# francis0407/streaming-benchmarks

Hardware: AMD Instinct MI355X
Metric: events/sec (parse+filter+join+window count) at 1/8 GPUs; % HBM roofline (higher is better)
Workload: dtype u8; 1 GPU; configs[1]: 100M JSON events per GPU, 100 campaigns x 10 ads, 10 s windows; events_per_gpu=100000000, campaigns=100, ads=1000, parallelism=1 GPU

## Files before the change

### streaming-benchmarks_amd/csrc/ysb_capi.cpp

```cpp
#include "ysb_ctx.h"

#include <unistd.h>

#include <cctype>

using namespace ysb;

thread_local std::string g_open_err;

int fail(ysb_ctx* c, int code, const char* fmt, ...) {
    char buf[1024];
    va_list ap;
    va_start(ap, fmt);
    vsnprintf(buf, sizeof buf, fmt, ap);
    va_end(ap);
    if (c) c->err = buf;
    else g_open_err = buf;
    return code;
}

int grow_device(ysb_ctx* c, DevMem& buf, u64 bytes, u64 floor_bytes) {
    if (buf.bytes() >= bytes) return YSB_OK;
    for (hipStream_t s : {c->s_comp, c->s_copy, c->s_split, c->s_x})
        if (s) HIPCHK(c, hipStreamSynchronize(s));
// ... 72 lines not shown
    c->max_ads = 1000;
    c->max_batch_events = 1u << 20;
    c->max_batch_bytes = 256ull << 20;
    c->ring_base_bucket = INT64_MIN;
    c->overflow_capacity = 1u << 20;
    c->flags = 0;
}

const char* ysb_last_error(const ysb_ctx* c) { return c ? c->err.c_str() : g_open_err.c_str(); }

static void destroy(ysb_ctx* c) {
    if (!c) return;
    hipSetDevice(c->device);
    for (hipStream_t s : {c->s_comp, c->s_copy, c->s_split, c->s_x})
        if (s) hipStreamSynchronize(s);
    if (c->comm) ncclCommDestroy(c->comm);
    for (auto& r : c->host_ranges) hipHostUnregister(reinterpret_cast<void*>(r.first));
    if (c->s_x) hipStreamDestroy(c->s_x);
    if (c->s_split) hipStreamDestroy(c->s_split);
    if (c->s_comp) hipStreamDestroy(c->s_comp);
    if (c->s_copy) hipStreamDestroy(c->s_copy);
    delete c;
}

static int init(ysb_ctx* c) {
    const ysb_config& cfg = c->cfg;
    if (hipSetDevice(c->device) != hipSuccess) return fail(c, YSB_ERR_HIP, "hipSetDevice(%d) failed", c->device);
    hipDeviceProp_t prop;
    if (hipGetDeviceProperties(&prop, c->device) == hipSuccess && prop.multiProcessorCount > 0) c->cus = prop.multiProcessorCount;
    if (const char* e = getenv("YSB_DYN_PCT")) c->dyn_pct = (u32)strtoul(e, nullptr, 10);
    if (const char* e = getenv("YSB_DELTA_FOLD_EVENTS")) {
        const u64 v = strtoull(e, nullptr, 10);
        if (v > 0 && v < c->delta_limit) c->delta_limit = v;
    }
    if (const char* e = getenv("YSB_DYN_CHUNK")) c->dyn_chunk = (u32)strtoul(e, nullptr, 10);
    if (const char* e = getenv("YSB_SPLIT_STREAM")) c->split_place = std::atoi(e);
    if (const char* e = getenv("YSB_H2D_WG")) c->h2d_wg = std::max(1, std::atoi(e));
    if (const char* e = getenv("YSB_H2D_PRIO")) c->h2d_prio = std::atoi(e) != 0;
    if (const char* e = getenv("YSB_H2D_GRID")) c->h2d_grid = std::max(0, std::atoi(e));
    if (hipStreamCreateWithFlags(&c->s_comp, hipStreamNonBlocking) != hipSuccess ||
        hipStreamCreateWithFlags(&c->s_copy, hipStreamNonBlocking) != hipSuccess)
        return fail(c, YSB_ERR_HIP, "stream creation failed");
    for (Event* e : {&c->ev_h2d[0], &c->ev_kdone[0], &c->ev_h2d[1], &c->ev_kdone[1], &c->ev_ring, &c->ev_used})
        if (e->create() != hipSuccess) return fail(c, YSB_ERR_HIP, "event creation failed");
    if (c->h_used.alloc(16) != hipSuccess) return fail(c, YSB_ERR_HIP, "event creation failed");
    const int rc = regrow_table(c, c->d_counts, 0, (u64)c->c_pad * cfg.window_ring);
    if (rc) return rc;
    c->side_slots = 64;
    while (c->side_slots < 2 * cfg.overflow_capacity) c->side_slots <<= 1;
    c->side_cbits = 1;
    while (c->side_cbits < 32 && (1ull << c->side_cbits) <= cfg.n_campaigns) ++c->side_cbits;
    if (c->d_side.alloc(c->side_slots * sizeof(SideSlot)) != hipSuccess ||
        c->d_stats.alloc((ST_COUNT_ + 1) * 8) != hipSuccess ||
        hipMemset(c->d_stats, 0, (ST_COUNT_ + 1) * 8) != hipSuccess ||
        c->d_dirty.alloc(16) != hipSuccess || hipMemset(c->d_dirty, 0, 16) != hipSuccess)
        return fail(c, YSB_ERR_NOMEM, "device allocation failed");
    c->d_side_used = reinterpret_cast<u32*>(c->d_stats + ST_COUNT_);
    launch_side_clear(c->d_side, c->side_slots, c->s_comp);
    if (hipStreamSynchronize(c->s_comp) != hipSuccess) return fail(c, YSB_ERR_HIP, "side map initialisation failed");
    if (c->d_ring.alloc(16) != hipSuccess || c->h_ring.alloc(16) != hipSuccess ||
        c->d_ovf.alloc(cfg.overflow_capacity * sizeof(OvfEntry)) != hipSuccess || c->d_ovf_count.alloc(16) != hipSuccess)
        return fail(c, YSB_ERR_NOMEM, "device allocation failed");
    i64 ring[2] = {0, 0};
    if (cfg.ring_base_bucket != INT64_MIN) {
        ring[0] = cfg.ring_base_bucket;
        ring[1] = 1;
// ... 570 lines not shown
```

### streaming-benchmarks_amd/csrc/ysb_count.hip

```cpp
#include "ysb_kernels.h"
#include <algorithm>

namespace ysb {

constexpr int REC_TPB = 1024;
constexpr int PART_RING = 32;
constexpr int REC_WAVES = REC_TPB / 64;
constexpr int REC_UNROLL = 8;
constexpr u32 REC_NONE = 0xFFFFFFFFu;

__global__ __launch_bounds__(REC_TPB) __attribute__((amdgpu_waves_per_eu(PART_RING == 32 ? 8 : 4)))
void rec_partition_kernel(const RecParams R) {
    __shared__ __attribute__((aligned(16))) u32 stage[REC_SUB_MAX * PART_RING];
    __shared__ u32 hist[REC_SUB_MAX];
    __shared__ u32 boff[REC_SUB_MAX];
    __shared__ u32 cur[REC_SUB_MAX];
    __shared__ u32 fl[REC_SUB_MAX];
    __shared__ u32 rounds_sh;
    const u32 tid = threadIdx.x, lane = tid & 63, wave = tid >> 6;
    const u32 b = blockIdx.x / REC_QUARTERS, q = blockIdx.x % REC_QUARTERS;
    const u32 S = 1u << R.sub_log2;
    for (u32 i = tid; i < S; i += REC_TPB) { hist[i] = 0; cur[i] = 0; fl[i] = 0; }
    if (tid == 0) rounds_sh = 0;
    const u32 w_lo = (u32)((u64)q * R.grid / REC_QUARTERS), w_hi = (u32)((u64)(q + 1) * R.grid / REC_QUARTERS);
    const u32 first_blk = b << R.sub_log2;
    const u32 sh = R.w_log2 + R.blk_shift;
    constexpr u32 CH = 64 * REC_UNROLL;
    u32 my_rounds = 0;
    for (u32 w = w_lo + wave; w < w_hi; w += REC_WAVES) my_rounds += (R.rec_n[(u64)w * R.bins + b] + CH - 1) / CH;
    __syncthreads();
    if (lane == 0) atomicMax(&rounds_sh, my_rounds);
    u32 cw = w_lo + wave, coff = 0, cn = cw < w_hi ? R.rec_n[(u64)cw * R.bins + b] : 0u;
    auto next_chunk = [&](u32 (&v)[REC_UNROLL]) {
        while (cw < w_hi && coff >= cn) {
            cw += REC_WAVES;
            coff = 0;
            cn = cw < w_hi ? R.rec_n[(u64)cw * R.bins + b] : 0u;
        }
        const u32* src = R.rec + ((u64)(cw < w_hi ? cw : w_lo) * R.bins + b) * R.cap;
#pragma unroll
        for (int u = 0; u < REC_UNROLL; ++u) {
            const u32 i = coff + u * 64 + lane;
// ... 49 lines not shown
            for (u32 j = 0; j < n; ++j) dst[j] = src[(f + j) & (PART_RING - 1)];
        }
        fl[k] = f + n;
    };
    cw = w_lo + wave;
    coff = 0;
    cn = cw < w_hi ? R.rec_n[(u64)cw * R.bins + b] : 0u;
    for (u32 r = 0; r < rounds; ++r) {
        if (r < my_rounds) {
            u32 v[REC_UNROLL];
            next_chunk(v);
#pragma unroll
            for (int u = 0; u < REC_UNROLL; ++u) {
                if (v[u] == REC_NONE) continue;
                const u32 k = (v[u] >> sh) - first_blk;
                const u32 pos = atomicAdd(&cur[k], 1u);
                if (pos - fl[k] < (u32)PART_RING) stage[k * PART_RING + (pos & (PART_RING - 1))] = v[u];
                else out[boff[k] + pos] = v[u];
            }
        }
        __syncthreads();
        for (u32 k = tid; k < S; k += REC_TPB) {
            const u32 f0 = fl[k], c = cur[k];
            const u32 lines = min(c - f0, (u32)PART_RING) / 32;
            for (u32 l = 0; l < lines; ++l) write_line(k, 32);
            if (c - f0 > (u32)PART_RING) fl[k] = c;
        }
        __syncthreads();
    }
    for (u32 k = tid; k < S; k += REC_TPB)
        if (cur[k] > fl[k]) write_line(k, cur[k] - fl[k]);
}

__device__ __forceinline__ uint4 add16(uint4 d, const u32* cnt16, unsigned long long* ring16, u32* dirty) {
    const u32 dw[4] = {d.x, d.y, d.z, d.w};
    u32 o[4];
#pragma unroll
    for (int k = 0; k < 4; ++k) {
        const uint4 c = reinterpret_cast<const uint4*>(cnt16)[k];
        const u32 cc[4] = {c.x, c.y, c.z, c.w};
        u32 w = 0;
#pragma unroll
        for (int j = 0; j < 4; ++j) {
            const u32 s = ((dw[k] >> (8 * j)) & 0xFFu) + cc[j];
            if (s > 255u) {
                atomicAdd(&ring16[4 * k + j], (unsigned long long)s);
                *dirty = 1u;
            } else {
                w |= s << (8 * j);
            }
        }
        o[k] = w;
    }
    return make_uint4(o[0], o[1], o[2], o[3]);
}

__global__ __launch_bounds__(REC_TPB) void rec_count_kernel(const RecParams R) {
    __shared__ __attribute__((aligned(16))) u32 cnt[REC_BLOCK_CELLS];
    __shared__ u32 roff[REC_QUARTERS + 1];
    __shared__ u32 rbeg[REC_QUARTERS];
    const u32 tid = threadIdx.x;
    const u32 j = blockIdx.x;
    const u32 c0 = j << R.blk_shift;
    const u32 nc = min(1u << R.blk_shift, R.c_pad - c0);
    const u32 cells = nc << R.w_log2;
    for (u32 i = tid; i < cells / 4; i += REC_TPB) reinterpret_cast<uint4*>(cnt)[i] = make_uint4(0, 0, 0, 0);
    if (tid < 64) {
        const u32 n = tid < (u32)REC_QUARTERS ? R.runs[((u64)j * REC_QUARTERS + tid) * 2 + 1] : 0u;
        if (tid < (u32)REC_QUARTERS) rbeg[tid] = R.runs[((u64)j * REC_QUARTERS + tid) * 2];
        u32 incl = n;
#pragma unroll
        for (int o = 1; o < 64; o <<= 1) {
            const u32 y = __shfl_up(incl, o, 64);
            if ((int)tid >= o) incl += y;
        }
        if (tid < (u32)REC_QUARTERS) roff[tid] = incl - n;
        if (tid == (u32)REC_QUARTERS - 1) roff[REC_QUARTERS] = incl;
    }
    __syncthreads();
    const u32 total = roff[REC_QUARTERS];
    const u32 base_cell = c0 << R.w_log2;
    uint4* dr = reinterpret_cast<uint4*>(R.delta + base_cell);
    const u32 quads = cells / 16;
    constexpr int SU = REC_BLOCK_CELLS / 16 / REC_TPB;
    static_assert(SU * REC_TPB * 16 == REC_BLOCK_CELLS, "one slab vector set per thread");
    unsigned long long* ring = R.counts + base_cell;
    const bool dense = (u64)total * 16u >= cells;
    uint4 r[SU];
    if (dense) {
#pragma unroll
        for (int u = 0; u < SU; ++u) {
            const u32 p = u * REC_TPB + tid;
            r[u] = p < quads ? dr[p] : make_uint4(0u, 0u, 0u, 0u);
        }
    }
    constexpr u32 TPS = REC_TPB / REC_QUARTERS;
    static_assert(TPS * REC_QUARTERS == REC_TPB && TPS >= 16, "one thread group per partition slice");
    const u32 q = tid / TPS, k = tid % TPS;
    const u32 nq = roff[q + 1] - roff[q];
    const u32* src = R.part + rbeg[q];
    for (u32 j0 = 0; j0 < nq; j0 += TPS * REC_UNROLL) {
        u32 v[REC_UNROLL];
#pragma unroll
        for (int u = 0; u < REC_UNROLL; ++u) {
            const u32 jj = j0 + u * TPS + k;
            v[u] = jj < nq ? src[jj] : REC_NONE;
        }
#pragma unroll
        for (int u = 0; u < REC_UNROLL; ++u)
            if (v[u] != REC_NONE) atomicAdd(&cnt[v[u] - base_cell], 1u);
    }
    __syncthreads();
    if (dense) {
#pragma unroll
        for (int u = 0; u < SU; ++u) {
            const u32 p = u * REC_TPB + tid;
            if (p < quads) dr[p] = add16(r[u], cnt + 16 * p, ring + 16 * (u64)p, R.dirty);
        }
        return;
    }
    bool live[SU];
#pragma unroll
    for (int u = 0; u < SU; ++u) {
        const u32 p = u * REC_TPB + tid;
        u32 any = 0;
        if (p < quads) {
#pragma unroll
            for (int j = 0; j < 4; ++j) {
                const uint4 c = reinterpret_cast<const uint4*>(cnt)[4 * p + j];
                any |= c.x | c.y | c.z | c.w;
            }
        }
        any |= __shfl_xor(any, 1, 64);
        any |= __shfl_xor(any, 2, 64);
        any |= __shfl_xor(any, 4, 64);
        live[u] = p < quads && any != 0u;
    }
#pragma unroll
    for (int u = 0; u < SU; ++u) {
        const u32 p = u * REC_TPB + tid;
        if (live[u]) r[u] = dr[p];
    }
#pragma unroll
    for (int u = 0; u < SU; ++u) {
        const u32 p = u * REC_TPB + tid;
        if (live[u]) dr[p] = add16(r[u], cnt + 16 * p, ring + 16 * (u64)p, R.dirty);
    }
}

__global__ __launch_bounds__(256) void fold_kernel(unsigned long long* counts, u8* delta, u64 vecs) {
    for (u64 q = (u64)blockIdx.x * 256 + threadIdx.x; q < vecs; q += (u64)gridDim.x * 256) {
        const uint4 d = reinterpret_cast<const uint4*>(delta)[q];
        if ((d.x | d.y | d.z | d.w) == 0u) continue;
        const u32 dw[4] = {d.x, d.y, d.z, d.w};
        ulonglong2* c2 = reinterpret_cast<ulonglong2*>(counts + 16 * q);
#pragma unroll
        for (int j = 0; j < 8; ++j) {
            if (((dw[j >> 1] >> (16 * (j & 1))) & 0xFFFFu) == 0u) continue;
            ulonglong2 a = c2[j];
            a.x += (dw[j >> 1] >> (16 * (j & 1))) & 0xFFu;
            a.y += (dw[j >> 1] >> (16 * (j & 1) + 8)) & 0xFFu;
            c2[j] = a;
        }
        reinterpret_cast<uint4*>(delta)[q] = make_uint4(0u, 0u, 0u, 0u);
    }
}

void launch_rec_partition(const RecParams& r, hipStream_t s) {
    hipLaunchKernelGGL(rec_partition_kernel, dim3(r.bins * REC_QUARTERS), dim3(REC_TPB), 0, s, r);
}

void launch_fold(unsigned long long* counts, u8* delta, u64 cells, hipStream_t s) {
    const u64 vecs = cells / 16;
    if (!vecs) return;
    const u64 blocks = std::min<u64>((vecs + 255) / 256, 65536);
    hipLaunchKernelGGL(fold_kernel, dim3((u32)blocks), dim3(256), 0, s, counts, delta, vecs);
}

void launch_rec_count(const RecParams& r, hipStream_t s) {
// ... 5 lines not shown
```

### streaming-benchmarks_amd/csrc/ysb_ctx.h

```cpp
#pragma once
#include <hip/hip_runtime.h>
#include <rccl/rccl.h>

#include <algorithm>
#include <array>
#include <cstdarg>
#include <cstdio>
#include <cstdlib>
#include <cstring>
#include <map>
#include <string>
#include <thread>
#include <utility>
#include <vector>

#include "../../include/ysb_hip.h"
#include "ysb_admap.h"
#include "ysb_kernels.h"
#include "ysb_layout.h"

using namespace ysb;


namespace ysb {
// ... 142 lines not shown
    DevBuf<i64> d_ring;
    PinBuf<i64> h_ring;
    Event ev_ring;
    bool ring_query_pending = false;
    bool ring_known = false;
    i64 ring_lo = 0;
    DevBuf<OvfEntry> d_ovf;
    DevBuf<u32> d_ovf_count;
    DevBuf<SideSlot> d_side;
    u64 side_slots = 0;
    u32 side_cbits = 1;
    u32* d_side_used = nullptr;
    DevBuf<unsigned long long> d_stats;
    u64 batches = 0;
    std::map<std::pair<u32, i64>, u64> side;
    DivMagic div{};
    u32 lds_wl = 0, lds_wl_log2 = 0;
    PinBuf<u8> h_bytes[2];
    PinBuf<u32> h_off[2];
    u8* hd_bytes[2] = {nullptr, nullptr};
    u32* hd_off[2] = {nullptr, nullptr};
    DevBuf<u8> d_bytes[2];
    DevBuf<u32> d_off[2];
    Event ev_h2d[2], ev_kdone[2];
    EventLog<3> tev;
    double path_ms_acc = 0;
    u64 path_launches_acc = 0;
    DevBuf<u32> d_rec, d_rec_n, d_part, d_runs;
    u64 rec_launches = 0;
    DevBuf<u8> d_delta;
    u64 delta_cells = 0;
    u64 delta_bound = 0;
    u64 delta_limit = ~0ull;
    bool pend_u64 = true;
    DevBuf<u32> d_dirty;
    ncclComm_t comm = nullptr;
    bool host_coll = false;
    ysb_collectives hops{};
    int rank = 0, nranks = 1;
    DevBuf<unsigned long long> d_xmax;
    PinBuf<unsigned long long> h_xmax;
    Event xplan_ev[2];
    int xb = 0;
    bool x_have_plan = false;
    hipStream_t s_x = nullptr;
    DevBuf<u32> d_xslots;
    DevBuf<void> d_xsend[2], d_xrecv[2];
    Event ev_xpacked[2], ev_xdone[2];
    bool xset_used[2] = {false, false};
    int xk = 0;
    int unpack_set = -1;
    u32 unpack_R = 0, unpack_width = 0;
    size_t unpack_entry = 0;
    u64 x_count = 0, x_bytes = 0;
    u32 x_last_slots = 0, x_last_width = 0;
    double x_ms = 0, x_crit_ms = 0, x_rs_ms = 0, x_exposed_ms = 0;
    std::vector<std::array<Event, 6>> xev;
    size_t xev_used = 0;
    struct FlushSlot {
        PinBuf<TableRow> h_rows;
        TableRow* hd_rows = nullptr;
        PinBuf<u32> h_n;
        u64 cap = 0;
        Event ev;
    };
    static constexpr int FLUSH_SLOTS = 4;
// ... 50 lines not shown
```

### streaming-benchmarks_amd/csrc/ysb_kernels.h

```cpp
#pragma once
#include <hip/hip_runtime.h>
#include "ysb_common.h"

namespace ysb {

constexpr int SCAN_TPB = 64;
#ifndef YSB_TILE_LINES
#define YSB_TILE_LINES 64
#endif
constexpr int TILE_LINES = YSB_TILE_LINES;
static_assert(TILE_LINES >= 1 && TILE_LINES <= SCAN_TPB, "one line per lane at most");
#ifndef YSB_WG_PER_CU
#define YSB_WG_PER_CU 8
#endif
#ifndef YSB_MAX_TILES
#define YSB_MAX_TILES 128
#endif
constexpr int SCAN_WG_PER_CU = YSB_WG_PER_CU;
#ifndef YSB_TILE_LINE_BYTES
#define YSB_TILE_LINE_BYTES 272
#endif
constexpr int TILE_CAP = TILE_LINES * YSB_TILE_LINE_BYTES;
constexpr int TILE_CHUNKS = TILE_CAP / 16;
constexpr int CHUNKS_PER_THREAD = (TILE_CHUNKS + SCAN_TPB - 1) / SCAN_TPB;
constexpr int LCNT_CAP = 256;
constexpr int MAX_TILES_PER_BLOCK = YSB_MAX_TILES;
#ifndef YSB_TBL_LINE_BYTES
#define YSB_TBL_LINE_BYTES 160
#endif
#ifndef YSB_TBL_WG_PER_CU
#define YSB_TBL_WG_PER_CU 12
#endif

constexpr int REC_BINS_MAX = 8;
constexpr int REC_RING = 64;
template <bool TBL, bool REC = false>
struct Geom {
    static constexpr int WG_PER_CU = TBL ? YSB_TBL_WG_PER_CU : SCAN_WG_PER_CU;
    static constexpr int CAP = TILE_LINES * (TBL ? YSB_TBL_LINE_BYTES - (REC ? 8 : 0) : YSB_TILE_LINE_BYTES);
    static constexpr int CHUNKS = CAP / 16;
    static constexpr int CPT = (CHUNKS + SCAN_TPB - 1) / SCAN_TPB;
    static constexpr int OFF_TILE = 0;
    static constexpr int OFF_LCNT = OFF_TILE + CAP + 64;
    static constexpr int LCNT_BYTES = REC ? REC_BINS_MAX * REC_RING * 4 : LCNT_CAP * 4;
    static constexpr int OFF_MISC = OFF_LCNT + LCNT_BYTES;
    static constexpr int OFF_TB = OFF_MISC + 64;
    static constexpr int LDS = OFF_TB + (MAX_TILES_PER_BLOCK + 4) * 4;
    static_assert(OFF_LCNT % 16 == 0 && OFF_MISC % 16 == 0 && OFF_TB % 16 == 0 && LDS % 16 == 0,
                  "LDS carve must stay 16-byte aligned");
    static constexpr int LDS_ALLOC = (LDS + 1279) / 1280 * 1280;
    static_assert(LDS_ALLOC * WG_PER_CU <= 163840, "WG_PER_CU workgroups must fit one CU's 160 KiB of LDS");
};
constexpr int AUX_TPB = 256;

constexpr int MAX_SEGS = 16;
struct ScanSeg {
    const u8* bytes;
    const u32* off;
    u64 n;
    u64 nbytes;
    u64 line_base;
    u64 n_tiles;
    u64 n_static;
    u32 tiles_per_block;
    u32 static_rem;
};

struct ScanParams {
// ... 48 lines not shown
    u32 shard_rank;
    u32 shard_n;
    u32* pend_dirty;
    u32* used_out;
    u32 learn_code;
    u32 learn_n;
    u32 learn_cp;
};

constexpr int REC_BLOCK_CELLS = 32768;
#ifndef YSB_REC_QUARTERS
#define YSB_REC_QUARTERS 64
#endif
constexpr int REC_QUARTERS = YSB_REC_QUARTERS;
constexpr int REC_SUB_MAX = 512;
struct RecParams {
    const u32* rec;
    const u32* rec_n;
    u32 grid;
    u32 bins;
    u32 cap;
    u32 sub_log2;
    u32 blk_shift;
    u32 n_blocks;
    u32 ring_w;
    u32 w_log2;
    u32 c_pad;
    u64 area;
    u32* part;
    u32* runs;
    u8* delta;
    unsigned long long* counts;
    u32* dirty;
};
void launch_rec_partition(const RecParams& r, hipStream_t s);
void launch_rec_count(const RecParams& r, hipStream_t s);
void launch_fold(unsigned long long* counts, u8* delta, u64 cells, hipStream_t s);

void launch_xplan(const unsigned long long* counts, const u8* delta, u32 W, u64 cells, int force_u64,
                  const u32* dirty, unsigned long long* slot_max, hipStream_t s);
void launch_xpack(unsigned long long* counts, u8* delta, u32 W, u32 rows, const u32* slots, u32 R, int force_u64,
                  const u32* dirty, void* out, u32 width, unsigned long long cap, hipStream_t s);
void launch_xunpack(unsigned long long* owned, u8* owned8, u32 W, u32 rows, const u32* slots, u32 R, const void* in,
                    u32 width, hipStream_t s);
void launch_checksum(const unsigned long long* table, u32 rows, u32 W, i64 ring_lo, u32 c_off, u32 c_lo, u32 c_hi,
                     unsigned long long* out, hipStream_t s);

u64 split_chunks(u64 nbytes);
void launch_h2d_copy(void* dst, const void* src, u64 bytes, int cus, hipStream_t s, bool prio = false);
void launch_h2d_copy_unaligned(void* dst, const void* src, u64 bytes, int wgs, hipStream_t s);
hipError_t launch_split_lines(const u8* b, u64 nbytes, u32* chunk, u32* off, u64 cap, unsigned long long* d_n,
                              hipStream_t s);
void launch_rebase(u8* b, u64 nbytes, const u32* off, u64 cap, const unsigned long long* d_n, u64 n_val,
                   const u32* tab, u64 tab_n, i64 lead, int cus, hipStream_t s);
struct SampleSegs {
    const u8* bytes[SAMPLE_MAX];
    const u32* off[SAMPLE_MAX];
    u64 nbytes[SAMPLE_MAX];
    u64 n[SAMPLE_MAX];
    u64 line[SAMPLE_MAX];
};
void launch_sample(const SampleSegs& s, u32 nseg, u8* out, hipStream_t st);

constexpr int N_STAMPS = 8;

void launch_scan(const ScanParams& p, hipStream_t s);
// ... 42 lines not shown
```

### streaming-benchmarks_amd/csrc/ysb_scan.hip

```cpp
#include <type_traits>

#include "ysb_kernels.h"

#ifndef YSB_DIAG_A_ONLY
#define YSB_DIAG_A_ONLY 0
#endif
#ifndef YSB_DIAG_NO_PROBE
#define YSB_DIAG_NO_PROBE 0
#endif
#ifndef YSB_DIAG_NO_PROBE2
#define YSB_DIAG_NO_PROBE2 0
#endif
#ifndef YSB_DIAG_NO_COUNT
#define YSB_DIAG_NO_COUNT 0
#endif
#ifndef YSB_DIAG_NO_REC
#define YSB_DIAG_NO_REC 0
#endif
#ifndef YSB_DIAG_NO_FLUSH
#define YSB_DIAG_NO_FLUSH 0
#endif
#ifndef YSB_DIAG_FLAT_IDX
#define YSB_DIAG_FLAT_IDX 0
#endif
// ... 392 lines not shown
        const u32 v = lcnt[i];
        if (v) {
            lcnt[i] = 0;
            if constexpr (!DIAG_NO_FLUSH)
                global_add(P, ring_lo, ring_set, i >> P.lds_wl_log2, lbase + (i64)(i & (WL - 1)), v, tl);
        }
    }
}

#ifdef YSB_STAMPS
#define STAMP_DECL unsigned long long st_acc[N_STAMPS] = {0}, st_last = stamp_now();
#define STAMP(i) do { const unsigned long long n_ = stamp_now(); st_acc[i] += n_ - st_last; st_last = n_; } while (0)
__device__ __forceinline__ unsigned long long stamp_now() {
    unsigned long long t;
    __builtin_amdgcn_sched_barrier(0);
    asm volatile("s_memtime %0\n\ts_waitcnt lgkmcnt(0)" : "=s"(t)::"memory");
    __builtin_amdgcn_sched_barrier(0);
    return t;
}
#else
#define STAMP_DECL
#define STAMP(i) do { } while (0)
#endif

__device__ __forceinline__ void rec_fallback(const ScanParams& P, u32 cell, i64 ring_lo, bool ring_set, Tally& tl) {
    const u32 wl2 = 31u - (u32)__builtin_clz(P.ring_w);
    const u32 c = cell >> wl2;
    const i64 slot = (i64)(cell & (P.ring_w - 1));
    const i64 b = ring_lo + ((slot - ring_lo) & (i64)(P.ring_w - 1));
    global_add(P, ring_lo, ring_set, c, b, 1u, tl);
    *P.pend_dirty = 1u;
}

__device__ __forceinline__ void rec_write(const ScanParams& P, const u32* ring, u32 b, u32 fl, u32 n, u32& gcur,
                                          int lane, i64 ring_lo, bool ring_set, Tally& tl) {
    const u32 g = (u32)__builtin_amdgcn_readlane((int)gcur, (int)b);
    const bool fits = g + n <= P.rec_cap;
    if ((u32)lane < n) {
        const u32 v = ring[b * REC_RING + ((fl + (u32)lane) & (REC_RING - 1))];
        if (fits) P.rec[((u64)blockIdx.x * P.rec_bins + b) * P.rec_cap + g + (u32)lane] = v;
        else rec_fallback(P, v, ring_lo, ring_set, tl);
    }
    if (fits && lane == (int)b) gcur = g + n;
}

template <bool SERIAL, bool TBL, bool REC, int LAY = 0>
__global__ __launch_bounds__(SCAN_TPB) __attribute__((amdgpu_waves_per_eu((Geom<TBL>::WG_PER_CU * SCAN_TPB + 255) / 256))) void scan_kernel(const ScanParams P0) {
    using G = Geom<TBL, REC>;
    constexpr int CPT = G::CPT;
    extern __shared__ __attribute__((aligned(16))) u8 smem[];
    u32* tile32 = reinterpret_cast<u32*>(smem + G::OFF_TILE);
    u32* lcnt = reinterpret_cast<u32*>(smem + G::OFF_LCNT);
    i64* misc64 = reinterpret_cast<i64*>(smem + G::OFF_MISC);
    u32* tb = reinterpret_cast<u32*>(smem + G::OFF_TB);
    u32* keytab = reinterpret_cast<u32*>(smem + G::LDS);
    if constexpr (!TBL && LAY >= 2) {
        if (threadIdx.x < 64) keytab[threadIdx.x] = KEYTAB.w[threadIdx.x];
        __syncthreads();
    }

    const int tid = threadIdx.x;
    const int lane = tid & 63;
#ifdef YSB_WGTIME
    const unsigned long long wg_t0 = __builtin_amdgcn_s_memrealtime();
#endif
    ScanParams P = P0;

    const i64 ring_lo = P.ring[0];
    const bool ring_set = P.ring[1] != 0;
    const u32 WL = P.lds_wl;
    const u32 ncells = WL ? P.n_campaigns * WL : 0u;
    for (u32 i = tid; i < ncells; i += SCAN_TPB) lcnt[i] = 0;
    u32* rcur = reinterpret_cast<u32*>(misc64);
    u32 gcur = 0;
    if (REC && tid < REC_BINS_MAX) rcur[tid] = 0;
    if (!REC && tid < 2) misc64[tid] = INT64_MIN;

    Tally tl{0, 0, 0, 0, 0, 0, 0, 0};
    constexpr int PF_DEPTH = 1;
    u64 t_begin = 0, t_end = 0, n_run = 0;
    TileInfo none{0, 0u, 0u, 0u, 0u, 0u, true};
    uint4 preA[CPT];
    u32 offA = 0, endA = 0;
    TileInfo infA = none;
    u32 tseq = 0;
    i64 lbase = 0;
    bool lset = false;

    const LdsSrc lsrc{tile32};
    const uint4* ct4 = reinterpret_cast<const uint4*>(P.ctable);
    if (blockIdx.x & 1) __builtin_amdgcn_s_setprio(1);
    STAMP_DECL
    auto tile_step = [&](u64 t, TileInfo& inf, uint4 (&pre)[CPT], u32& pre_off, u32& pre_end) {
        const TileInfo cur = inf;
        const u32 my_off = pre_off;
        const u32 li = lane_line(tid);
        const u32 my_end = (cur.first + li + 1 < P.n) ? pre_end : (u32)P.nbytes;
#ifdef YSB_STAMPS
        asm volatile("s_waitcnt vmcnt(0)" ::: "memory");
        STAMP(6);
#endif
        if (!cur.oversize) {
#pragma unroll
            for (int j = 0; j < CPT; ++j) {
                const u32 k = (u32)(j * SCAN_TPB + tid);
                if (j * SCAN_TPB + SCAN_TPB <= G::CHUNKS || k < (u32)G::CHUNKS) {
                    reinterpret_cast<uint4*>(tile32)[k] = pre[j];
                }
            }
        }
        const int par = (int)(tseq++ & 1);
        if (WL) {
            const i64 req = misc64[par ^ 1];
            if (req != INT64_MIN) {
                if (lset) flush_window(P, lcnt, ncells, WL, lbase, ring_lo, ring_set, tl);
                lbase = req - (i64)(WL / 2) + 1;
                lset = true;
            }
        }
        STAMP(0);
        __syncthreads();
        if (!REC && tid == 0) misc64[par ^ 1] = INT64_MIN;
        STAMP(1);
        if constexpr (DIAG_A_ONLY) {
            inf = t + PF_DEPTH < t_end ? tile_info<G::CAP>(P, t + PF_DEPTH, t_begin, tb) : none;
            issue_tile_loads(P.bytes, P.off, P.n, li, inf, pre, pre_off, pre_end);
            __syncthreads();
            return;
        }
        bool ok1 = false, elig = false;
        int ls = 0, le = 0;
        CanonA ca;
#pragma unroll
        for (int k = 0; k < 9; ++k) ca.kw[k] = 0u;
        ca.t0 = 0;
        CanonB cb;
        cb.view = false;
        if (li < cur.count && !cur.oversize && my_off >= cur.s0 && my_end >= my_off && my_end <= cur.e) {
            elig = true;
            ls = (int)(my_off - cur.s0 + cur.delta);
            le = (int)(my_end - cur.s0 + cur.delta);
            if constexpr (TBL) ok1 = tbl_stage1(lsrc, ls, le, ca);
            else if constexpr (LAY == 2 && DIAG_FLAT_IDX) {
                const u32 x = flat_index_only(lsrc, ls, le);
                if (x == 0x9E3779B9u) tl.miss += 1;
            }
            else if constexpr (LAY == 2) ok1 = flat_tier<LdsSrc, true>(lsrc, ls, le, P.require_mask, ca, cb, keytab);
            else if constexpr (LAY == 3) {
                ok1 = P.learn_cp ? learned_parse<true>(lsrc, ls, le, P, ca, cb) : learned_parse<false>(lsrc, ls, le, P, ca, cb);
                if (__builtin_expect(!ok1, 0)) ok1 = flat_tier<LdsSrc, true>(lsrc, ls, le, P.require_mask, ca, cb, keytab);
            }
            else if constexpr (LAY == 4) {}
            else ok1 = vocab_stage1<LAY == 1>(lsrc, ls, le, ca);
        }
        int mode = 0;
        bool fl = false;
        if constexpr (LAY == 4) {
            u32 cls = 0;
            if (elig) {
                const u32 h2 = lsrc.load4(ls + 8);
                const bool up = lsrc.load4(ls) == w4('{', '"', 'u', 's') && lsrc.load4(ls + 4) == w4('e', 'r', '_', 'i') &&
                                (h2 & 0xFFFFFFu) == (w4('d', '"', ':', 0) & 0xFFFFFFu);
                cls = up && (h2 >> 24) == ' ' ? 1u : up && (h2 >> 24) == '"' ? 2u : 3u;
            }
            const u64 b1 = __ballot(cls == 1u), b2 = __ballot(cls == 2u), b3 = __ballot(cls == 3u);
            mode = (b2 | b3) == 0ull ? 1 : (b1 | b3) == 0ull ? 2 : ((b1 | b2) == 0ull && P.learn_n) ? 3 : 4;
            if (elig) {
                if (mode == 1) ok1 = vocab_stage1<false>(lsrc, ls, le, ca);
                else if (mode == 2) ok1 = vocab_stage1<true>(lsrc, ls, le, ca);
                else if (mode == 3) {
                    ok1 = P.learn_cp ? learned_parse<true>(lsrc, ls, le, P, ca, cb) : learned_parse<false>(lsrc, ls, le, P, ca, cb);
                    fl = !ok1;
                } else {
                    fl = true;
                }
            }
        }
        bool pend = false, dfr = false, tok = false;
        i64 bucket = 0;
        bool ok2 = false;
        if (li < cur.count) {
            if constexpr (TBL) ok2 = ok1 && tbl_stage2(lsrc, ls, le, ca, cb);
            else if constexpr (LAY == 2 || LAY == 3) ok2 = ok1;
            else if constexpr (LAY == 4) {
                if (mode == 1) ok2 = ok1 && vocab_stage2<false>(lsrc, ls, le, ca, cb);
                else if (mode == 2) ok2 = ok1 && vocab_stage2<true>(lsrc, ls, le, ca, cb);
                else ok2 = ok1;
                if (mode <= 2) fl = elig && !ok2;
            }
            else ok2 = ok1 && vocab_stage2<LAY == 1>(lsrc, ls, le, ca, cb);
        }
        if constexpr (!TBL && LAY < 2) {
            if (__builtin_expect(elig && !ok2, 0)) {
                CanonA c2;
                CanonB b2;
                b2.view = false;
                const u32 h2 = lsrc.load4(ls + 8);
                const bool up = lsrc.load4(ls) == w4('{', '"', 'u', 's') && lsrc.load4(ls + 4) == w4('e', 'r', '_', 'i') &&
                                (h2 & 0xFFFFFFu) == (w4('d', '"', ':', 0) & 0xFFFFFFu);
                bool t = false;
                if constexpr (LAY == 1) {
                    if (up && (h2 >> 24) == ' ') {
                        t = vocab_stage1<false>(lsrc, ls, le, c2) && vocab_stage2<false>(lsrc, ls, le, c2, b2);
                        if (!t) t = canon_stage1<false>(lsrc, ls, le, c2) && canon_stage2<false>(lsrc, ls, le, c2, b2);
                    } else if (up && (h2 >> 24) == '"') {
                        t = canon_stage1<true>(lsrc, ls, le, c2) && canon_stage2<true>(lsrc, ls, le, c2, b2);
                    }
                } else {
                if (up && (h2 >> 24) == ' ')
// ... 30 lines not shown
#pragma unroll
        for (int j = 0; j < (int)CB_Q; ++j) q[j] = a0;
        u32 ib_s = 0;
        if constexpr (DIAG_NO_PROBE) {
            if (pend) {
                a0 = make_uint4(ca.kw[0], ca.kw[1], ca.kw[2], ca.kw[3]);
                a1 = make_uint4(ca.kw[4], ca.kw[5], ca.kw[6], ca.kw[7]);
                a2 = make_uint4(ca.kw[8], ca.kw[0] % P.n_campaigns, 0, 0);
                q[0] = a0;
                q[1] = a1;
                q[2] = a2;
            }
        }
        if (pend && !DIAG_NO_PROBE) {
            u32 ia, ib;
            cuckoo_slots36(ca.kw, P.cseed, P.ctable_mask, &ia, &ib);
            if constexpr (SERIAL) {
#pragma unroll
                for (int j = 0; j < (int)CB_Q; ++j) q[j] = ct4[CB_Q * (u64)ia + j];
                ib_s = ib;
            } else {
                a0 = ct4[CSLOT_Q * (u64)ia]; a1 = ct4[CSLOT_Q * (u64)ia + 1]; a2 = ct4[CSLOT_Q * (u64)ia + 2];
                b0 = ct4[CSLOT_Q * (u64)ib]; b1 = ct4[CSLOT_Q * (u64)ib + 1]; b2 = ct4[CSLOT_Q * (u64)ib + 2];
            }
        }
        if (ok2) {
            tl.ev++;
            if (pend) {
                tl.view++;
                tok = canonical_bucket<TBL>(lsrc, cb, ls + ca.t0, P, bucket);
            }
        }
        defer_append(P, dfr, P.line_base + cur.first + li, lane);
        STAMP(2);
        inf = t + PF_DEPTH < t_end ? tile_info<G::CAP>(P, t + PF_DEPTH, t_begin, tb) : none;
        issue_tile_loads(P.bytes, P.off, P.n, li, inf, pre, pre_off, pre_end);
        bool valid = false, dfr2 = false;
        u32 campaign = 0;
        if (pend) {
            const u32* k = ca.kw;
            u32 ci;
            if constexpr (SERIAL) {
                bool full;
                ci = bucket_find(q, k, full);
                if (!DIAG_NO_PROBE2 && ci == EMPTY_SLOT && full) {
#pragma unroll
                    for (int j = 0; j < (int)CB_Q; ++j) q[j] = ct4[CB_Q * (u64)ib_s + j];
                    ci = bucket_find(q, k, full);
                }
            } else {
                const u32 da = (a0.x ^ k[0]) | (a0.y ^ k[1]) | (a0.z ^ k[2]) | (a0.w ^ k[3]) | (a1.x ^ k[4]) |
                               (a1.y ^ k[5]) | (a1.z ^ k[6]) | (a1.w ^ k[7]) | (a2.x ^ k[8]);
                const u32 db = (b0.x ^ k[0]) | (b0.y ^ k[1]) | (b0.z ^ k[2]) | (b0.w ^ k[3]) | (b1.x ^ k[4]) |
                               (b1.y ^ k[5]) | (b1.z ^ k[6]) | (b1.w ^ k[7]) | (b2.x ^ k[8]);
                ci = (da == 0u && a2.y != EMPTY_SLOT) ? a2.y : (db == 0u ? b2.y : EMPTY_SLOT);
            }
            if (ci == EMPTY_SLOT) {
                if (P.ctable_partial) {
                    dfr2 = true;
                    tl.ev--;
                    tl.view--;
                } else {
                    tl.miss++;
                }
            } else {
                tl.join++;
                campaign = ci;
                valid = tok;
                if (!tok) tl.terr++;
            }
        }
        if (P.ctable_partial) defer_append(P, dfr2, P.line_base + cur.first + li, lane);
        STAMP(3);
        bool rec_has = false;
        u32 rec_bin = 0, rec_val = 0;
        if (WL) {
            if (valid) {
                const i64 rel = bucket - lbase;
                if (lset && rel >= 0 && rel < (i64)WL) {
                    atomicAdd(&lcnt[(campaign << P.lds_wl_log2) + (u32)rel], 1u);
                } else {
                    global_add(P, ring_lo, ring_set, campaign, bucket, 1u, tl);
                    if (!lset || rel >= (i64)WL) atomicMax(reinterpret_cast<long long*>(&misc64[par]), (long long)bucket);
                }
            }
        } else if (valid && !DIAG_NO_COUNT) {
            if constexpr (REC) {
                const i64 rel = bucket - ring_lo;
                if (ring_set && rel >= 0 && rel < (i64)P.ring_w) {
                    rec_has = true;
                    rec_bin = campaign >> P.rec_shift;
                    rec_val = campaign * P.ring_w + (u32)(bucket & (i64)(P.ring_w - 1));
                } else {
                    global_add(P, ring_lo, ring_set, campaign, bucket, 1u, tl);
                }
            } else {
                global_add(P, ring_lo, ring_set, campaign, bucket, 1u, tl);
            }
        }
        if constexpr (DIAG_NO_REC) rec_has = false;
        if constexpr (REC) {
#pragma unroll
            for (int half = 0; half < 2; ++half) {
                const bool mine = rec_has && (tid >> 5) == half;
                u32 pos = 0;
                if (mine) {
                    pos = atomicAdd(&rcur[rec_bin], 1u);
                    lcnt[rec_bin * REC_RING + (pos & (REC_RING - 1))] = rec_val;
                }
                unsigned long long done = __ballot(mine && (pos & 31u) == 31u);
                while (done) {
                    const int src = (int)__builtin_ctzll(done);
                    done &= done - 1;
                    const u32 b = (u32)__builtin_amdgcn_readlane((int)rec_bin, src);
                    const u32 p = (u32)__builtin_amdgcn_readlane((int)pos, src);
                    rec_write(P, lcnt, b, p - 31u, 32u, gcur, lane, ring_lo, ring_set, tl);
                }
            }
        }
        STAMP(4);
        __syncthreads();
        STAMP(5);
    };
    auto run_tiles = [&]() {
        n_run += t_end - t_begin;
        for (u32 i = tid; i <= (u32)(t_end - t_begin); i += SCAN_TPB) {
            const u64 f = (t_begin + i) * TILE_LINES;
            tb[i] = f < P.n ? P.off[f] : (u32)P.nbytes;
        }
        __syncthreads();
        infA = tile_info<G::CAP>(P, t_begin, t_begin, tb);
        issue_tile_loads(P.bytes, P.off, P.n, lane_line(tid), infA, preA, offA, endA);
        for (u64 t = t_begin; t < t_end; ++t) tile_step(t, infA, preA, offA, endA);
    };
    auto use_segment = [&](const ScanSeg& sg) {
        P.bytes = sg.bytes;
        P.off = sg.off;
        P.n = sg.n;
        P.nbytes = sg.nbytes;
        P.line_base = sg.line_base;
        none.first = sg.n;
    };
    const u64 wg = blockIdx.x;
    for (u32 sgi = 0; sgi < P0.n_segs; ++sgi) {
        const ScanSeg& sg = P0.seg[sgi];
        t_begin = wg * sg.tiles_per_block + (wg < sg.static_rem ? wg : (u64)sg.static_rem);
        t_end = t_begin + sg.tiles_per_block + (wg < sg.static_rem ? 1u : 0u);
        if (t_begin >= t_end) continue;
        use_segment(sg);
        run_tiles();
    }
    if (P0.dyn_chunk) {
        u32 sgi = 0;
        u32 claim = 0;
        auto claim_next = [&](u32 si) -> u32 {
            u32 c = 0;
            if (lane == 0) c = atomicAdd(&P0.dyn_ctr[si], 1u);
            return c;
        };
        while (sgi < P0.n_segs && P0.seg[sgi].n_static >= P0.seg[sgi].n_tiles) ++sgi;
        if (sgi < P0.n_segs) claim = claim_next(sgi);
        while (sgi < P0.n_segs) {
            const ScanSeg& sg = P0.seg[sgi];
            const u32 c = (u32)__builtin_amdgcn_readfirstlane(__shfl(claim, 0, 64));
            t_begin = sg.n_static + (u64)c * P0.dyn_chunk;
            if (t_begin >= sg.n_tiles) {
                ++sgi;
                while (sgi < P0.n_segs && P0.seg[sgi].n_static >= P0.seg[sgi].n_tiles) ++sgi;
                if (sgi < P0.n_segs) claim = claim_next(sgi);
                continue;
            }
            t_end = min<u64>(t_begin + P0.dyn_chunk, sg.n_tiles);
            claim = claim_next(sgi);
            use_segment(sg);
            run_tiles();
        }
    }
    if constexpr (REC) {
        for (u32 b = 0; b < P.rec_bins; ++b) {
            const u32 staged = rcur[b], n = staged & 31u;
            if (n) rec_write(P, lcnt, b, staged - n, n, gcur, lane, ring_lo, ring_set, tl);
        }
        if (tid < (int)P.rec_bins) P.rec_n[(u64)blockIdx.x * P.rec_bins + tid] = gcur;
    }
    if (n_run == 0) return;
#ifdef YSB_STAMPS
    if (lane == 0) {
        unsigned long long* o = P.dbg + ((u64)blockIdx.x * (SCAN_TPB / 64) + (threadIdx.x >> 6)) * N_STAMPS;
        for (int i = 0; i < 7; ++i) o[i] += st_acc[i];
        o[7] += n_run;
    }
#endif
    if (WL && lset) flush_window(P, lcnt, ncells, WL, lbase, ring_lo, ring_set, tl);
    flush_tally(P, tl, lane);
#ifdef YSB_WGTIME
    if (lane == 0) {
        unsigned long long* o = P.dbg + (u64)blockIdx.x * N_STAMPS;
        o[0] = wg_t0;
        o[1] = __builtin_amdgcn_s_memrealtime();
        o[2] = n_run;
    }
#endif
}

template <class S>
__device__ __forceinline__ int tbl_split(const S& src, int s, int& e, int (&p)[6]) {
    if (e > s && src.b(e - 1) == '\n') --e;
    if (e > s && src.b(e - 1) == '\r') --e;
    int k = 0;
    for (int q = s; q < e && k < 6; ++q)
        if (src.b(q) == '|') p[k++] = q;
// ... 198 lines not shown
```

### streaming-benchmarks_amd/csrc/ysb_submit.cpp

```cpp
#include "ysb_ctx.h"

using namespace ysb;

extern "C" {


struct Layout {
    int layout = -1;
    LearnDesc learn{};
};

static u32 require_mask(const ysb_ctx* c) { return (c->cfg.flags & YSB_F_REQUIRE_IP) ? 0x7Fu : 0x3Fu; }
static bool flat_first(const ysb_ctx* c) { return (c->cfg.flags & YSB_F_FLAT_FIRST) != 0; }

static ScanParams make_params(ysb_ctx* c, const ysb_segment* segs, u32 nseg, const Layout& lay) {
    ScanParams p{};
    p.tbl = (c->cfg.flags & YSB_F_FORMAT_TBL) ? 1u : 0u;
    p.bytes = segs[0].d_bytes;
    p.nbytes = segs[0].nbytes;
    p.off = segs[0].d_line_off;
    p.n = segs[0].n_events;
    p.line_base = 0;
    p.table = c->d_table;
    p.table_mask = (u32)(c->table_slots - 1);
// ... 84 lines not shown
    const u32 sub = (r.n_blocks + REC_BINS_MAX - 1) / REC_BINS_MAX;
    r.sub_log2 = log2u(sub);
    if ((1u << r.sub_log2) > (u32)REC_SUB_MAX) return YSB_OK;
    r.bins = (r.n_blocks + (1u << r.sub_log2) - 1) >> r.sub_log2;
    r.grid = p.grid;
    if ((r.grid + REC_QUARTERS - 1) / REC_QUARTERS > 128) return YSB_OK;
    u64 tiles = 0;
    for (u32 i = 0; i < p.n_segs; ++i) tiles += p.seg[i].tiles_per_block + (p.seg[i].static_rem ? 1 : 0);
    const u64 lines = tiles * TILE_LINES;
    u64 cap = (lines * 3 / 4 + r.bins - 1) / r.bins;
    cap = std::max<u64>(32, (cap + 31) / 32 * 32);
    const u64 area = ((u64)((r.grid + REC_QUARTERS - 1) / REC_QUARTERS) * cap + 32ull * (1u << r.sub_log2) + 31) / 32 * 32;
    const u64 part = (u64)r.bins * REC_QUARTERS * area;
    if (cap > 0xFFFFFFFFull || part >= (1ull << 32)) return YSB_OK;
    r.cap = (u32)cap;
    r.area = area;
    int rc;
    if ((rc = grow_device(c, c->d_rec, (u64)r.grid * r.bins * cap * 4, 0))) return rc;
    if ((rc = grow_device(c, c->d_rec_n, (u64)r.grid * r.bins * 4, 0))) return rc;
    if ((rc = grow_device(c, c->d_part, part * 4, 0))) return rc;
    if ((rc = grow_device(c, c->d_runs, (u64)r.n_blocks * REC_QUARTERS * 2 * 4, 0))) return rc;
    if (c->delta_cells != cells) {
        if ((rc = fold_delta(c))) return rc;
        c->delta_cells = 0;
        if ((rc = grow_device(c, c->d_delta, cells, 0))) return rc;
        HIPCHK(c, hipMemset(c->d_delta, 0, cells));
        c->delta_cells = cells;
    }
    if (c->delta_bound + n_events >= c->delta_limit && (rc = fold_delta(c))) return rc;
    c->delta_bound += n_events;
    r.delta = c->d_delta;
    r.counts = c->d_counts;
    r.dirty = c->d_dirty;
    r.rec = c->d_rec;
    r.rec_n = c->d_rec_n;
    r.part = c->d_part;
    r.runs = c->d_runs;
    p.rec_on = 1;
    p.rec_bins = r.bins;
    p.rec_shift = r.blk_shift + r.sub_log2;
    p.rec_cap = r.cap;
    p.rec = c->d_rec;
    p.rec_n = c->d_rec_n;
    return YSB_OK;
}

static int enqueue_scan(ysb_ctx* c, const ysb_segment* in, u32 nin, const Layout& lay) {
    if (!c->table_loaded) return fail(c, YSB_ERR_STATE, "ysb_load_ad_map has not been called");
    ysb_segment segs[MAX_SEGS];
    u32 nseg = 0;
    u64 n = 0;
    for (u32 i = 0; i < nin; ++i)
        if (in[i].n_events) { segs[nseg++] = in[i]; n += in[i].n_events; }
    if (n == 0) { c->batches += nin; return YSB_OK; }
    if (n >= (1ull << 31)) return fail(c, YSB_ERR_CAPACITY, "at most 2^31-1 events per launch");
    int rc = grow_device(c, c->d_defer, n * 4, 4u << 16);
    if (rc) return rc;
    if (!c->d_defer_ctr) {
        HIPCHK(c, c->d_defer_ctr.alloc(16 + 4 * MAX_SEGS));
        HIPCHK(c, hipMemset(c->d_defer_ctr, 0, 16 + 4 * MAX_SEGS));
    }
    if (c->used_pending && hipEventQuery(c->ev_used) == hipSuccess) {
        c->used_pending = false;
        if ((u64)*c->h_used * 4 > c->side_slots) {
            rc = sync_streams(c);
            if (!rc) rc = pull_side_list(c);
// ... 549 lines not shown
```

Before: 24.98 billion events/s.

## Pack record counters to u16 in LDS and defer record staging across tile steps

The count kernel now keeps two 16-bit counters per LDS word, halving shared memory so more waves fit per EU (waves_per_eu 8). Blocks whose record total could overflow 16 bits fall back to a two-pass split over halves with full 32-bit counters. Separately, the scan kernel carries each tile's record into the next tile step and spreads the LDS staging atomics, ring placement and global stores across phases of that step, to overlap them with parsing work. This adds complexity and extra barriers in the split path, and the carried record state must be drained correctly at the end.

```diff
diff --git a/streaming-benchmarks_amd/csrc/ysb_capi.cpp b/streaming-benchmarks_amd/csrc/ysb_capi.cpp
--- a/streaming-benchmarks_amd/csrc/ysb_capi.cpp
+++ b/streaming-benchmarks_amd/csrc/ysb_capi.cpp
@@ -128,6 +128,10 @@
     if (const char* e = getenv("YSB_DELTA_FOLD_EVENTS")) {
         const u64 v = strtoull(e, nullptr, 10);
         if (v > 0 && v < c->delta_limit) c->delta_limit = v;
+    }
+    if (const char* e = getenv("YSB_REC_U16_LIMIT")) {
+        const u64 v = strtoull(e, nullptr, 10);
+        if (v > 0 && v < c->rec_u16_limit) c->rec_u16_limit = (u32)v;
     }
     if (const char* e = getenv("YSB_DYN_CHUNK")) c->dyn_chunk = (u32)strtoul(e, nullptr, 10);
     if (const char* e = getenv("YSB_SPLIT_STREAM")) c->split_place = std::atoi(e);
diff --git a/streaming-benchmarks_amd/csrc/ysb_count.hip b/streaming-benchmarks_amd/csrc/ysb_count.hip
--- a/streaming-benchmarks_amd/csrc/ysb_count.hip
+++ b/streaming-benchmarks_amd/csrc/ysb_count.hip
@@ -7,7 +7,6 @@
 constexpr int PART_RING = 32;
 constexpr int REC_WAVES = REC_TPB / 64;
 constexpr int REC_UNROLL = 8;
-constexpr u32 REC_NONE = 0xFFFFFFFFu;
 
 __global__ __launch_bounds__(REC_TPB) __attribute__((amdgpu_waves_per_eu(PART_RING == 32 ? 8 : 4)))
 void rec_partition_kernel(const RecParams R) {
@@ -123,13 +122,25 @@
         if (cur[k] > fl[k]) write_line(k, cur[k] - fl[k]);
 }
 
+template <bool PACKED>
 __device__ __forceinline__ uint4 add16(uint4 d, const u32* cnt16, unsigned long long* ring16, u32* dirty) {
     const u32 dw[4] = {d.x, d.y, d.z, d.w};
     u32 o[4];
+    uint4 pk[2];
+    if constexpr (PACKED) {
+        pk[0] = reinterpret_cast<const uint4*>(cnt16)[0];
+        pk[1] = reinterpret_cast<const uint4*>(cnt16)[1];
+    }
 #pragma unroll
     for (int k = 0; k < 4; ++k) {
-        const uint4 c = reinterpret_cast<const uint4*>(cnt16)[k];
-        const u32 cc[4] = {c.x, c.y, c.z, c.w};
+        u32 cc[4];
+        if constexpr (PACKED) {
+            const u32 lo = (k & 1) ? pk[k >> 1].z : pk[k >> 1].x, hi = (k & 1) ? pk[k >> 1].w : pk[k >> 1].y;
+            cc[0] = lo & 0xFFFFu; cc[1] = lo >> 16; cc[2] = hi & 0xFFFFu; cc[3] = hi >> 16;
+        } else {
+            const uint4 c = reinterpret_cast<const uint4*>(cnt16)[k];
+            cc[0] = c.x; cc[1] = c.y; cc[2] = c.z; cc[3] = c.w;
+        }
         u32 w = 0;
 #pragma unroll
         for (int j = 0; j < 4; ++j) {
@@ -146,8 +157,10 @@
     return make_uint4(o[0], o[1], o[2], o[3]);
 }
 
-__global__ __launch_bounds__(REC_TPB) void rec_count_kernel(const RecParams R) {
-    __shared__ __attribute__((aligned(16))) u32 cnt[REC_BLOCK_CELLS];
+__global__ __launch_bounds__(REC_TPB) __attribute__((amdgpu_waves_per_eu(8)))
+void rec_count_kernel(const RecParams R) {
+    constexpr u32 CNT_WORDS = REC_BLOCK_CELLS / 2;
+    __shared__ __attribute__((aligned(16))) u32 cnt[CNT_WORDS];
     __shared__ u32 roff[REC_QUARTERS + 1];
     __shared__ u32 rbeg[REC_QUARTERS];
     const u32 tid = threadIdx.x;
@@ -155,7 +168,7 @@
     const u32 c0 = j << R.blk_shift;
     const u32 nc = min(1u << R.blk_shift, R.c_pad - c0);
     const u32 cells = nc << R.w_log2;
-    for (u32 i = tid; i < cells / 4; i += REC_TPB) reinterpret_cast<uint4*>(cnt)[i] = make_uint4(0, 0, 0, 0);
+    for (u32 i = tid; i < cells / 8; i += REC_TPB) reinterpret_cast<uint4*>(cnt)[i] = make_uint4(0, 0, 0, 0);
     if (tid < 64) {
         const u32 n = tid < (u32)REC_QUARTERS ? R.runs[((u64)j * REC_QUARTERS + tid) * 2 + 1] : 0u;
         if (tid < (u32)REC_QUARTERS) rbeg[tid] = R.runs[((u64)j * REC_QUARTERS + tid) * 2];
@@ -176,7 +189,8 @@
     constexpr int SU = REC_BLOCK_CELLS / 16 / REC_TPB;
     static_assert(SU * REC_TPB * 16 == REC_BLOCK_CELLS, "one slab vector set per thread");
     unsigned long long* ring = R.counts + base_cell;
-    const bool dense = (u64)total * 16u >= cells;
+    const bool split = total >= R.u16_limit;
+    const bool dense = !split && (u64)total * 16u >= cells;
     uint4 r[SU];
     if (dense) {
 #pragma unroll
@@ -190,23 +204,43 @@
     const u32 q = tid / TPS, k = tid % TPS;
     const u32 nq = roff[q + 1] - roff[q];
     const u32* src = R.part + rbeg[q];
-    for (u32 j0 = 0; j0 < nq; j0 += TPS * REC_UNROLL) {
-        u32 v[REC_UNROLL];
-#pragma unroll
-        for (int u = 0; u < REC_UNROLL; ++u) {
-            const u32 jj = j0 + u * TPS + k;
-            v[u] = jj < nq ? src[jj] : REC_NONE;
-        }
-#pragma unroll
-        for (int u = 0; u < REC_UNROLL; ++u)
-            if (v[u] != REC_NONE) atomicAdd(&cnt[v[u] - base_cell], 1u);
-    }
+    auto for_records = [&](auto&& count) {
+        for (u32 j0 = 0; j0 < nq; j0 += TPS * REC_UNROLL) {
+            u32 v[REC_UNROLL];
+#pragma unroll
+            for (int u = 0; u < REC_UNROLL; ++u) {
+                const u32 jj = j0 + u * TPS + k;
+                v[u] = jj < nq ? src[jj] : REC_NONE;
+            }
+#pragma unroll
+            for (int u = 0; u < REC_UNROLL; ++u)
+                if (v[u] != REC_NONE) count(v[u] - base_cell);
+        }
+    };
+    if (split) {
+        constexpr u32 HALF = CNT_WORDS;
+        for (u32 h0 = 0; h0 < cells; h0 += HALF) {
+            const u32 hc = min(HALF, cells - h0);
+            __syncthreads();
+            for (u32 i = tid; i < hc / 4; i += REC_TPB) reinterpret_cast<uint4*>(cnt)[i] = make_uint4(0, 0, 0, 0);
+            __syncthreads();
+            for_records([&](u32 x) { if (x - h0 < hc) atomicAdd(&cnt[x - h0], 1u); });
+            __syncthreads();
+            for (u32 p = tid; p < hc / 16; p += REC_TPB) {
+                const u32 pp = h0 / 16 + p;
+                dr[pp] = add16<false>(dr[pp], cnt + 16 * p, ring + 16 * (u64)pp, R.dirty);
+            }
+        }
+        return;
+    }
+    constexpr u32 QW = 8;
+    for_records([&](u32 x) { atomicAdd(&cnt[x >> 1], 1u << (16 * (x & 1))); });
     __syncthreads();
     if (dense) {
 #pragma unroll
         for (int u = 0; u < SU; ++u) {
             const u32 p = u * REC_TPB + tid;
-            if (p < quads) dr[p] = add16(r[u], cnt + 16 * p, ring + 16 * (u64)p, R.dirty);
+            if (p < quads) dr[p] = add16<true>(r[u], cnt + QW * p, ring + 16 * (u64)p, R.dirty);
         }
         return;
     }
@@ -217,8 +251,8 @@
         u32 any = 0;
         if (p < quads) {
 #pragma unroll
-            for (int j = 0; j < 4; ++j) {
-                const uint4 c = reinterpret_cast<const uint4*>(cnt)[4 * p + j];
+            for (int j = 0; j < (int)QW / 4; ++j) {
+                const uint4 c = reinterpret_cast<const uint4*>(cnt)[QW / 4 * p + j];
                 any |= c.x | c.y | c.z | c.w;
             }
         }
@@ -235,7 +269,7 @@
 #pragma unroll
     for (int u = 0; u < SU; ++u) {
         const u32 p = u * REC_TPB + tid;
-        if (live[u]) dr[p] = add16(r[u], cnt + 16 * p, ring + 16 * (u64)p, R.dirty);
+        if (live[u]) dr[p] = add16<true>(r[u], cnt + QW * p, ring + 16 * (u64)p, R.dirty);
     }
 }
 
diff --git a/streaming-benchmarks_amd/csrc/ysb_ctx.h b/streaming-benchmarks_amd/csrc/ysb_ctx.h
--- a/streaming-benchmarks_amd/csrc/ysb_ctx.h
+++ b/streaming-benchmarks_amd/csrc/ysb_ctx.h
@@ -198,6 +198,7 @@
     u64 delta_cells = 0;
     u64 delta_bound = 0;
     u64 delta_limit = ~0ull;
+    u32 rec_u16_limit = 65536;
     bool pend_u64 = true;
     DevBuf<u32> d_dirty;
     ncclComm_t comm = nullptr;
diff --git a/streaming-benchmarks_amd/csrc/ysb_kernels.h b/streaming-benchmarks_amd/csrc/ysb_kernels.h
--- a/streaming-benchmarks_amd/csrc/ysb_kernels.h
+++ b/streaming-benchmarks_amd/csrc/ysb_kernels.h
@@ -34,6 +34,7 @@
 
 constexpr int REC_BINS_MAX = 8;
 constexpr int REC_RING = 64;
+constexpr u32 REC_NONE = 0xFFFFFFFFu;
 template <bool TBL, bool REC = false>
 struct Geom {
     static constexpr int WG_PER_CU = TBL ? YSB_TBL_WG_PER_CU : SCAN_WG_PER_CU;
@@ -148,6 +149,7 @@
     u8* delta;
     unsigned long long* counts;
     u32* dirty;
+    u32 u16_limit;
 };
 void launch_rec_partition(const RecParams& r, hipStream_t s);
 void launch_rec_count(const RecParams& r, hipStream_t s);
diff --git a/streaming-benchmarks_amd/csrc/ysb_scan.hip b/streaming-benchmarks_amd/csrc/ysb_scan.hip
--- a/streaming-benchmarks_amd/csrc/ysb_scan.hip
+++ b/streaming-benchmarks_amd/csrc/ysb_scan.hip
@@ -448,16 +448,22 @@
     *P.pend_dirty = 1u;
 }
 
-__device__ __forceinline__ void rec_write(const ScanParams& P, const u32* ring, u32 b, u32 fl, u32 n, u32& gcur,
-                                          int lane, i64 ring_lo, bool ring_set, Tally& tl) {
+__device__ __forceinline__ u32 rec_read(const u32* ring, u32 b, u32 fl, u32 n, int lane) {
+    return (u32)lane < n ? ring[b * REC_RING + ((fl + (u32)lane) & (REC_RING - 1))] : 0u;
+}
+__device__ __forceinline__ void rec_store(const ScanParams& P, u32 b, u32 n, u32 v, u32& gcur, int lane, i64 ring_lo,
+                                          bool ring_set, Tally& tl) {
     const u32 g = (u32)__builtin_amdgcn_readlane((int)gcur, (int)b);
     const bool fits = g + n <= P.rec_cap;
     if ((u32)lane < n) {
-        const u32 v = ring[b * REC_RING + ((fl + (u32)lane) & (REC_RING - 1))];
         if (fits) P.rec[((u64)blockIdx.x * P.rec_bins + b) * P.rec_cap + g + (u32)lane] = v;
         else rec_fallback(P, v, ring_lo, ring_set, tl);
     }
     if (fits && lane == (int)b) gcur = g + n;
+}
+__device__ __forceinline__ void rec_write(const ScanParams& P, const u32* ring, u32 b, u32 fl, u32 n, u32& gcur,
+                                          int lane, i64 ring_lo, bool ring_set, Tally& tl) {
+    rec_store(P, b, n, rec_read(ring, b, fl, n, lane), gcur, lane, ring_lo, ring_set, tl);
 }
 
 template <bool SERIAL, bool TBL, bool REC, int LAY = 0>
@@ -490,6 +496,8 @@
     u32* rcur = reinterpret_cast<u32*>(misc64);
     u32 gcur = 0;
     if (REC && tid < REC_BINS_MAX) rcur[tid] = 0;
+    u32 carry = REC_NONE;
+    const u32 rec_bin_sh = REC ? 31u - (u32)__builtin_clz(P0.ring_w) + P0.rec_shift : 0u;
     if (!REC && tid < 2) misc64[tid] = INT64_MIN;
 
     Tally tl{0, 0, 0, 0, 0, 0, 0, 0};
@@ -507,6 +515,31 @@
     const uint4* ct4 = reinterpret_cast<const uint4*>(P.ctable);
     if (blockIdx.x & 1) __builtin_amdgcn_s_setprio(1);
     STAMP_DECL
+    auto stage_issue = [&](int half, u32& pos) {
+        if (carry != REC_NONE && (tid >> 5) == half) pos = atomicAdd(&rcur[carry >> rec_bin_sh], 1u);
+    };
+    auto stage_place = [&](int half, u32 pos, u32& lv, u32& lb) {
+        const bool mine = carry != REC_NONE && (tid >> 5) == half;
+        const u32 bin = carry >> rec_bin_sh;
+        if (mine) lcnt[bin * REC_RING + (pos & (REC_RING - 1))] = carry;
+        unsigned long long done = __ballot(mine && (pos & 31u) == 31u);
+        lb = REC_NONE;
+        while (done) {
+            const int src = (int)__builtin_ctzll(done);
+            done &= done - 1;
+            const u32 b = (u32)__builtin_amdgcn_readlane((int)bin, src);
+            const u32 p = (u32)__builtin_amdgcn_readlane((int)pos, src);
+            if (lb == REC_NONE) {
+                lb = b;
+                lv = rec_read(lcnt, b, p - 31u, 32u, lane);
+            } else {
+                rec_write(P, lcnt, b, p - 31u, 32u, gcur, lane, ring_lo, ring_set, tl);
+            }
+        }
+    };
+    auto stage_store = [&](u32 lv, u32 lb) {
+        if (lb != REC_NONE) rec_store(P, lb, 32u, lv, gcur, lane, ring_lo, ring_set, tl);
+    };
     auto tile_step = [&](u64 t, TileInfo& inf, uint4 (&pre)[CPT], u32& pre_off, u32& pre_end) {
         const TileInfo cur = inf;
         const u32 my_off = pre_off;
@@ -516,6 +549,7 @@
         asm volatile("s_waitcnt vmcnt(0)" ::: "memory");
         STAMP(6);
 #endif
+        u32 pos0 = 0, pos1 = 0, lv0 = 0, lv1 = 0, lb0 = REC_NONE, lb1 = REC_NONE;
         if (!cur.oversize) {
 #pragma unroll
             for (int j = 0; j < CPT; ++j) {
@@ -534,6 +568,7 @@
                 lset = true;
             }
         }
+        if constexpr (REC) stage_issue(0, pos0);
         STAMP(0);
         __syncthreads();
         if (!REC && tid == 0) misc64[par ^ 1] = INT64_MIN;
@@ -543,6 +578,10 @@
             issue_tile_loads(P.bytes, P.off, P.n, li, inf, pre, pre_off, pre_end);
             __syncthreads();
             return;
+        }
+        if constexpr (REC) {
+            stage_place(0, pos0, lv0, lb0);
+            stage_issue(1, pos1);
         }
         bool ok1 = false, elig = false;
         int ls = 0, le = 0;
@@ -591,6 +630,10 @@
                     fl = true;
                 }
             }
+        }
+        if constexpr (REC) {
+            stage_store(lv0, lb0);
+            stage_place(1, pos1, lv1, lb1);
         }
         bool pend = false, dfr = false, tok = false;
         i64 bucket = 0;
@@ -687,6 +730,7 @@
             }
         }
         defer_append(P, dfr, P.line_base + cur.first + li, lane);
+        if constexpr (REC) stage_store(lv1, lb1);
         STAMP(2);
         inf = t + PF_DEPTH < t_end ? tile_info<G::CAP>(P, t + PF_DEPTH, t_begin, tb) : none;
         issue_tile_loads(P.bytes, P.off, P.n, li, inf, pre, pre_off, pre_end);
@@ -728,7 +772,7 @@
         if (P.ctable_partial) defer_append(P, dfr2, P.line_base + cur.first + li, lane);
         STAMP(3);
         bool rec_has = false;
-        u32 rec_bin = 0, rec_val = 0;
+        u32 rec_val = 0;
         if (WL) {
             if (valid) {
                 const i64 rel = bucket - lbase;
@@ -744,7 +788,6 @@
                 const i64 rel = bucket - ring_lo;
                 if (ring_set && rel >= 0 && rel < (i64)P.ring_w) {
                     rec_has = true;
-                    rec_bin = campaign >> P.rec_shift;
                     rec_val = campaign * P.ring_w + (u32)(bucket & (i64)(P.ring_w - 1));
                 } else {
                     global_add(P, ring_lo, ring_set, campaign, bucket, 1u, tl);
@@ -754,25 +797,7 @@
             }
         }
         if constexpr (DIAG_NO_REC) rec_has = false;
-        if constexpr (REC) {
-#pragma unroll
-            for (int half = 0; half < 2; ++half) {
-                const bool mine = rec_has && (tid >> 5) == half;
-                u32 pos = 0;
-                if (mine) {
-                    pos = atomicAdd(&rcur[rec_bin], 1u);
-                    lcnt[rec_bin * REC_RING + (pos & (REC_RING - 1))] = rec_val;
-                }
-                unsigned long long done = __ballot(mine && (pos & 31u) == 31u);
-                while (done) {
-                    const int src = (int)__builtin_ctzll(done);
-                    done &= done - 1;
-                    const u32 b = (u32)__builtin_amdgcn_readlane((int)rec_bin, src);
-                    const u32 p = (u32)__builtin_amdgcn_readlane((int)pos, src);
-                    rec_write(P, lcnt, b, p - 31u, 32u, gcur, lane, ring_lo, ring_set, tl);
-                }
-            }
-        }
+        if constexpr (REC) carry = rec_has ? rec_val : REC_NONE;
         STAMP(4);
         __syncthreads();
         STAMP(5);
@@ -832,6 +857,15 @@
         }
     }
     if constexpr (REC) {
+#pragma unroll 1
+        for (int half = 0; half < 2; ++half) {
+            u32 pos = 0, lv = 0, lb = REC_NONE;
+            stage_issue(half, pos);
+            stage_place(half, pos, lv, lb);
+            stage_store(lv, lb);
+        }
+        carry = REC_NONE;
+        __syncthreads();
         for (u32 b = 0; b < P.rec_bins; ++b) {
             const u32 staged = rcur[b], n = staged & 31u;
             if (n) rec_write(P, lcnt, b, staged - n, n, gcur, lane, ring_lo, ring_set, tl);
diff --git a/streaming-benchmarks_amd/csrc/ysb_submit.cpp b/streaming-benchmarks_amd/csrc/ysb_submit.cpp
--- a/streaming-benchmarks_amd/csrc/ysb_submit.cpp
+++ b/streaming-benchmarks_amd/csrc/ysb_submit.cpp
@@ -140,6 +140,7 @@
     r.delta = c->d_delta;
     r.counts = c->d_counts;
     r.dirty = c->d_dirty;
+    r.u16_limit = c->rec_u16_limit;
     r.rec = c->d_rec;
     r.rec_n = c->d_rec_n;
     r.part = c->d_part;
```

New measurement: 24.95 billion events/s. About the same (-0.1%).
